# bkram/fmtuner-sdr

Measured on AMD Instinct MI355X. Metric: IQ MS/s demodulated per GPU (2.4 MS/s FM channels, stereo+RDS) at 1/2/4/8 MI355X, higher is better.
Workload: dtype f32 (FIR operands f16 hi+lo, f32 accumulate)

## Files before the change

fmtuner-sdr_amd/csrc/fmx_kernels.hip:

```cpp
#include <hip/hip_ext.h>
#include <hip/hip_fp16.h>
#include <hip/hip_runtime.h>

#include <cstddef>
#include <type_traits>

#include "fmx_internal.h"
#include "fmx_math.h"
#include "fmx_synth.h"


namespace fmx {

#define FE_T 768
#define FE_HALO_IQ 120
#define AU_T 768
#define AU_HALO 120
#define AU_RHALO 32
#define AU_MAXOUT 256

static constexpr float kPiF = 3.14159265358979323846f;

#define FMX_CONST __attribute__((address_space(4)))
template <typename T> __device__ __forceinline__ const FMX_CONST T *cptr(const T *p) {
// ... 743 lines not shown
      }
      keep[cntk++] = v;
    }
    __syncthreads();
    cntk = 0;
    uint8_t *dh = a.dec_hist + (size_t)c * 2 * FMX_MAX_DEC;
    for (int h = tid; h < L - 1; h += 256) {
      const uint16_t v = keep[cntk++];
      dh[2 * h] = (uint8_t)(v & 255);
      dh[2 * h + 1] = (uint8_t)(v >> 8);
    }
    if (tid == 0) {
      long nv = (long)dec_valid + total;
      a.dec_valid[c] = (int)(nv > (L - 1) ? (L - 1) : nv);
    }
  }
  if (demod) {
    for (int h = tid; h < FE_HALO_IQ; h += 256) {
      const float2 v = xin[h];
      a.iq_hist[(size_t)c * (FMX_IQ_MAXLEN - 1) + h] = float2_t{v.x, v.y};
    }
    if (tid == 0) {
      a.dc_v[2 * c] = sh->carry_i;
      a.dc_v[2 * c + 1] = sh->carry_q;
      a.fd_prev[2 * c] = sh->fd_re;
      a.fd_prev[2 * c + 1] = sh->fd_im;
      if (par.agc != 0) {
        a.agc[2 * c] = agc_g;
        a.agc[2 * c + 1] = agc_y2p;
      }
    }
  }
  if (hist_out) {
    float *hist = a.st_hist_wr + (size_t)c * FMX_HIST;
    for (int h = tid; h < FMX_HIST; h += 256) hist[h] = mx[h];
  }
  if (rds) {
    if (tid < 32) a.rds_hist[(size_t)c * 32 + tid] = rb[tid];
    if (tid == 0) a.rds_count[c] = sched_n;
  }
  FE_STAMP(6)
#ifdef FMX_STAMPS
  if (a.dbg && tid == 0)
    for (int k = 0; k < 8; ++k) atomicAdd(a.dbg + k, st_acc[k]);
#endif
#undef FE_STAMP
  if (tid == 0 && a.clip_out && a.in_mode != FE_IN_MPX)
    a.clip_out[c] = (n > 0) ? (float)sh->clip / (float)n : 0.0f;
  if (want_sig) fe_signal_sums(a, sig, sgp, c, lane, wave, tid);
}

__device__ __forceinline__ void dma_dword(const float *src, uint32_t lds) {
  unsigned keep;
  asm volatile("s_mov_b32 %0, m0\n\ts_mov_b32 m0, %2\n\ts_nop 0\n\tglobal_load_lds_dword %1, off\n\ts_mov_b32 m0, %0"
               : "=&s"(keep)
               : "v"(src), "s"(__builtin_amdgcn_readfirstlane(lds))
               : "memory");
}
__device__ __forceinline__ void dma_dword_s(const float *base, uint32_t voff, uint32_t lds) {
  __builtin_amdgcn_global_load_lds(reinterpret_cast<const char *>(base) + voff,
                                   (__attribute__((address_space(3))) void *)(uintptr_t)__builtin_amdgcn_readfirstlane(lds), 4, 0, 0);
}
__device__ __forceinline__ void dma_dwordx3(const float *src, uint32_t lds) {
  unsigned keep;
  asm volatile("s_mov_b32 %0, m0\n\ts_mov_b32 m0, %2\n\ts_nop 0\n\tglobal_load_lds_dwordx3 %1, off\n\ts_mov_b32 m0, %0"
               : "=&s"(keep)
               : "v"(src), "s"(__builtin_amdgcn_readfirstlane(lds))
               : "memory");
}
__device__ __forceinline__ uint32_t lds_addr(const void *p) {
  return __builtin_amdgcn_readfirstlane((uint32_t)(uintptr_t)(const __attribute__((address_space(3))) char *)p);
}
__device__ __forceinline__ void word_sincos(uint32_t theta, float *s, float *c) { fmx_word_sincos(theta, s, c); }

#include "fmx_pll.inc"

#define AU2_T 2048
#define AU2_PT 8
#define AU2_MAXOUT (AU2_T / 3 + 16)
#define AU_IMG (AU_HALO + AU2_T + 24)
#define AU_FN (AU_RHALO + AU2_T)
struct AuShared {
  float2 xf[AU_IMG > AU_FN ? AU_IMG : AU_FN] __attribute__((aligned(16)));
  float2 fh[AU_RHALO];
  float2 o[AU2_MAXOUT];
  float hT[FMX_AF_SUB][FMX_NPFB];
  float2 hf[AU_HALO];
  float ws[3][4][2];
  float iir[4];
  int eb, ee, count;
  uint32_t lrq[((2 * FMX_LR_QN + 63) / 64) * 64] __attribute__((aligned(16)));
};

template <int CTRL, int ROWS> __device__ __forceinline__ float dpp_or(float x, float id) {
  return __builtin_bit_cast(float, __builtin_amdgcn_update_dpp(__builtin_bit_cast(int, id), __builtin_bit_cast(int, x), CTRL,
                                                               ROWS, 0xF, false));
}
#define WAVE_AFF_STEP(CTRL, ROWS)                                                       \
  {                                                                                   \
    const float pA_ = dpp_or<CTRL, ROWS>(A, 1.0f), p1_ = dpp_or<CTRL, ROWS>(B1, 0.0f); \
    const float p2_ = dpp_or<CTRL, ROWS>(B2, 0.0f);                                     \
    B1 = A * p1_ + B1;                                                                \
    B2 = A * p2_ + B2;                                                                \
    A = A * pA_;                                                                      \
  }
__device__ __forceinline__ void wave_affine_scan(float &A, float &B1, float &B2) {
  WAVE_AFF_STEP(0x111, 0xF)
  WAVE_AFF_STEP(0x112, 0xF)
  WAVE_AFF_STEP(0x114, 0xF)
  WAVE_AFF_STEP(0x118, 0xF)
  WAVE_AFF_STEP(0x142, 0xA)
  WAVE_AFF_STEP(0x143, 0xC)
}
#undef WAVE_AFF_STEP
__device__ __forceinline__ void wave_affine_prev(float A, float B1, float B2, float &eA, float &e1, float &e2) {
  eA = dpp_or<0x138, 0xF>(A, 1.0f);
  e1 = dpp_or<0x138, 0xF>(B1, 0.0f);
  e2 = dpp_or<0x138, 0xF>(B2, 0.0f);
}

__device__ __forceinline__ void au_scan_prev(float A, float BL, float BR, float cl, float cr, float (*ws)[4][2],
                                             float &pl, float &pr) {
  const int tid = threadIdx.x, lane = tid & 63, wave = tid >> 6;
  wave_affine_scan(A, BL, BR);
  if (lane == 63) {
    ws[0][wave][0] = A;
    ws[1][wave][0] = BL;
    ws[2][wave][0] = BR;
  }
  float eA, eL, eR;
  wave_affine_prev(A, BL, BR, eA, eL, eR);
  __syncthreads();
  float vl = cl, vr = cr;
  for (int w = 0; w < wave; ++w) {
    vl = ws[0][w][0] * vl + ws[1][w][0];
    vr = ws[0][w][0] * vr + ws[2][w][0];
  }
  pl = eA * vl + eL;
  pr = eA * vr + eR;
  __syncthreads();
}

#ifndef FMX_AU_WPE
#define FMX_AU_WPE 1
#endif
__global__ __launch_bounds__(256) __attribute__((amdgpu_waves_per_eu(FMX_AU_WPE))) void k_audio(AudioArgs a) {
  extern __shared__ __align__(16) unsigned char au_smem[];
  AuShared &S = *reinterpret_cast<AuShared *>(au_smem);
  const int c = au_channel(blockIdx.x, a.C, a.in_tiled != 0);
  const int tid = threadIdx.x;
  const FmxDesign *__restrict__ D = a.des;
  const FmxChanParam par = a.par[c];
  const int n = a.n;
  const bool mono = (a.mode == 2 || a.mode == 3);
  const bool lrfir = (a.mode == 0 || a.mode == 4);
  const bool af = (a.mode != 4);
  const bool pipe_mono = (a.mode == 3);
  const int deemph = par.deemph;
  const float dalpha = (deemph == 0) ? D->deemph_alpha[0] : ((deemph == 1) ? D->deemph_alpha[1] : par.deemph_alpha);
  const bool de_on = deemph != 2;
  const float dc_alpha = mono ? 0.0008f : 0.005f;
  const float de_a1 = -(1.0f - dalpha);
  const float dc_a1 = -1.0f + dc_alpha;
  if (a.sig_out && blockIdx.x * 256 < (unsigned)a.C) {
    const int cs = blockIdx.x * 256 + tid;
    if (cs < a.C)
      signal_level_eval(a.sig_sums + 6 * (size_t)cs, a.sig_samples, a.sig_par + 4 * (size_t)cs,
                        a.sig_smooth + 2 * (size_t)cs, a.sig_out + cs);
  }
  float *lrh = a.lr_hist + (size_t)c * 2 * (FMX_LR_LEN - 1);
  float *win = mono ? a.mono_win + (size_t)c * 32 : a.af_win + (size_t)c * 2 * 32;
  float2 *const F = S.xf;
  float2 cx = make_float2(0.0f, 0.0f);
  if (lrfir && tid < AU_HALO) cx = make_float2(lrh[tid], lrh[(FMX_LR_LEN - 1) + tid]);
  if (af)
    for (int h = tid; h < AU_RHALO; h += 256) S.fh[h] = make_float2(win[h], mono ? 0.0f : win[32 + h]);
  float *iir = mono ? a.mono_iir + (size_t)c * 2 : a.af_iir + (size_t)c * 4;
  if (af && tid == 0) {
    if (mono) {
      S.iir[0] = iir[0];
      S.iir[1] = 0.0f;
      S.iir[2] = iir[1];
      S.iir[3] = 0.0f;
    } else {
      for (int k = 0; k < 4; ++k) S.iir[k] = iir[k];
    }
  }
  const FmxSched *sched = nullptr;
  int sched_n = 0;
  if (af) {
    const int g = a.group[c];
    sched = a.sched + (size_t)g * a.sched_stride;
    sched_n = a.sched_n[g];
    for (int k = tid; k < FMX_NPFB * FMX_AF_SUB; k += 256) {
      const int b = k / FMX_AF_SUB, nn = k % FMX_AF_SUB;
      S.hT[nn][b] = D->af_h[k];
    }
  }
  if (lrfir) {
    static_assert(FMX_LR_QN % 2 == 0, "dword window");
    const float *qs = reinterpret_cast<const float *>(&D->lr_q16[0][0][0]);
    for (int p = tid >> 6; p < (2 * FMX_LR_QN + 63) / 64; p += 4)
      dma_dword(qs + min(64 * p + (tid & 63), 2 * FMX_LR_QN - 1), lds_addr(&S.lrq[64 * p]));
  }
  if (tid == 0) {
    S.eb = 0;
    S.count = 0;
  }
  const bool tiled = a.in_tiled != 0;
  const float *inl = a.in_l + (tiled ? lr_tile_idx(c, 0, a.in_stride) : (size_t)c * a.in_stride);
  const float *inr = mono ? nullptr : a.in_r + (tiled ? lr_tile_idx(c, 0, a.in_stride) : (size_t)c * a.in_stride);
  auto ti = [&](int j) __attribute__((always_inline)) { return tiled ? (j >> 4) * 32 + (j & 15) : j; };
  const float sc = D->lr_scale;
  int mrem = 0, mtot = 0;
  if (a.mute) {
    mrem = a.mute[2 * c];
    mtot = a.mute[2 * c + 1];
  }
  const int mdone = (mtot > mrem) ? mtot - mrem : 0;
  const int mfade = max(1, min(a.mute_fade, mtot / 2));
  __syncthreads();
  for (int n0 = 0; n0 < n; n0 += AU2_T) {
    const int cnt = min(AU2_T, n - n0);
    FmxSched en3[3];
    if (af) {
      const int eb = S.eb;
#pragma unroll
      for (int k = 0; k < 3; ++k) {
        const int e = eb + tid + 256 * k;
        en3[k] = (e < sched_n) ? sched[e] : FmxSched{0xFFFF, 0.0f};
      }
    }
    {
      float vl[AU2_PT], vr[AU2_PT];
#pragma unroll
      for (int k = 0; k < AU2_PT; ++k) {
        const int j = tid + 256 * k;
        vl[k] = (j < cnt) ? inl[ti(n0 + j)] : 0.0f;
        vr[k] = (j < cnt && !mono) ? inr[ti(n0 + j)] : 0.0f;
      }
      if (lrfir) {
        _Float16 *im = reinterpret_cast<_Float16 *>(S.xf);
        auto put = [&](int i, float l, float r) __attribute__((always_inline)) {
          l *= 1024.0f;
          r *= 1024.0f;
          const _Float16 lh = (_Float16)l, rh = (_Float16)r;
          im[i] = lh;
          im[AU_IMG + i] = (_Float16)(l - (float)lh);
          im[2 * AU_IMG + i] = rh;
          im[3 * AU_IMG + i] = (_Float16)(r - (float)rh);
        };
        if (tid < AU_HALO) put(tid, cx.x, cx.y);
#pragma unroll
        for (int k = 0; k < AU2_PT; ++k) put(AU_HALO + tid + 256 * k, vl[k], vr[k]);
        if (tid < AU_IMG - AU_HALO - AU2_T) put(AU_HALO + AU2_T + tid, 0.0f, 0.0f);
#pragma unroll
        for (int k = 0; k < AU2_PT; ++k) {
          const int j = tid + 256 * k;
          if (j >= cnt - AU_HALO && j < cnt) S.hf[j - (cnt - AU_HALO)] = make_float2(vl[k], vr[k]);
        }
        if (tid < AU_HALO && tid >= cnt) S.hf[tid - cnt] = cx;
      } else {
#pragma unroll
        for (int k = 0; k < AU2_PT; ++k) {
          const int j = tid + 256 * k;
          if (j < cnt) F[AU_RHALO + j] = make_float2(vl[k], vr[k]);
        }
      }
      if (!lrfir && af && tid < AU_RHALO) F[tid] = S.fh[tid];
    }
    if (tid == 0) S.ee = S.eb;
    __syncthreads();
    if (lrfir) {
      typedef _Float16 f16x8_t __attribute__((ext_vector_type(8)));
      typedef float f32x4_t __attribute__((ext_vector_type(4)));
      typedef unsigned int u32x4 __attribute__((ext_vector_type(4)));
      const int lane = tid & 63, wave = tid >> 6, col = lane & 15, g = lane >> 4;
      const _Float16 *im = reinterpret_cast<const _Float16 *>(S.xf);
      const int xb = 16 * (32 * wave + col) + 8 * g;
      const f16x8_t *bLh = reinterpret_cast<const f16x8_t *>(im + xb);
      const f16x8_t *bLl = reinterpret_cast<const f16x8_t *>(im + AU_IMG + xb);
      const f16x8_t *bRh = reinterpret_cast<const f16x8_t *>(im + 2 * AU_IMG + xb);
      const f16x8_t *bRl = reinterpret_cast<const f16x8_t *>(im + 3 * AU_IMG + xb);
      const int qb = 8 * g + 15 - col, qc = qb & 1;
      const uint32_t *qh = &S.lrq[0] + qc * FMX_LR_QN + (qb - qc) / 2;
      const uint32_t *ql = qh + FMX_LR_QN / 2;
      auto frag = [&](int ks, const uint32_t *q) __attribute__((always_inline)) {
        return u32x4{q[16 * ks], q[16 * ks + 1], q[16 * ks + 2], q[16 * ks + 3]};
      };
      f32x4_t aL[2], aR[2];
      aL[0] = aL[1] = aR[0] = aR[1] = f32x4_t{0.0f, 0.0f, 0.0f, 0.0f};
      u32x4 ah = frag(0, qh), al = frag(0, ql);
#pragma unroll
      for (int ks = 0; ks < FMX_LR_KS; ++ks) {
        const f16x8_t ahi = __builtin_bit_cast(f16x8_t, ah), alo = __builtin_bit_cast(f16x8_t, al);
        if (ks + 1 < FMX_LR_KS) {
          ah = frag(ks + 1, qh);
          al = frag(ks + 1, ql);
        }
#pragma unroll
        for (int u = 0; u < 2; ++u) {
          const f16x8_t lh = bLh[32 * u + 4 * ks], ll = bLl[32 * u + 4 * ks];
          const f16x8_t rh = bRh[32 * u + 4 * ks], rl = bRl[32 * u + 4 * ks];
          aL[u] = __builtin_amdgcn_mfma_f32_16x16x32_f16(lh, ahi, aL[u], 0, 0, 0);
          aR[u] = __builtin_amdgcn_mfma_f32_16x16x32_f16(rh, ahi, aR[u], 0, 0, 0);
          aL[u] = __builtin_amdgcn_mfma_f32_16x16x32_f16(ll, ahi, aL[u], 0, 0, 0);
          aR[u] = __builtin_amdgcn_mfma_f32_16x16x32_f16(rl, ahi, aR[u], 0, 0, 0);
          aL[u] = __builtin_amdgcn_mfma_f32_16x16x32_f16(lh, alo, aL[u], 0, 0, 0);
          aR[u] = __builtin_amdgcn_mfma_f32_16x16x32_f16(rh, alo, aR[u], 0, 0, 0);
        }
      }
      if (tid < AU_HALO) cx = S.hf[tid];
      __syncthreads();
      if (af && tid < AU_RHALO) F[tid] = S.fh[tid];
      const float osc = sc * (1.0f / 4194304.0f);
#pragma unroll
      for (int u = 0; u < 2; ++u) {
#pragma unroll
        for (int i = 0; i < 4; ++i) {
          const int j = 256 * (2 * wave + u) + 16 * (4 * g + i) + col;
          const float2 y = make_float2(aL[u][i] * osc, aR[u][i] * osc);
          if (af) F[AU_RHALO + j] = y;
          if (a.lr_out_l && j < cnt) {
            a.lr_out_l[(size_t)c * a.lr_out_stride + n0 + j] = y.x;
            a.lr_out_r[(size_t)c * a.lr_out_stride + n0 + j] = y.y;
          }
        }
      }
    }
    __syncthreads();
    if (af) {
      const int eb = S.eb;
      int last = -1;
#pragma unroll
      for (int k = 0; k < 3; ++k) {
        const int e = eb + tid + 256 * k;
        if (e < sched_n && (en3[k].packed & 0xFFFF) < n0 + cnt) {
          const int i = (en3[k].packed & 0xFFFF) - n0;
          const int b = (en3[k].packed >> 16) & 0xFF;
          const bool boundary = (en3[k].packed >> 24) & 1;
          const int b0 = boundary ? FMX_NPFB - 1 : b, b1 = boundary ? 0 : b + 1;
          const int i0 = boundary ? i - 1 : i;
          float y0l = 0.0f, y0r = 0.0f, y1l = 0.0f, y1r = 0.0f;
          auto mac = [](float &y, float h, float x) __attribute__((always_inline)) {
            float t;
            asm("v_mul_f32 %0, %2, %3\n\tv_add_f32 %1, %1, %0" : "=&v"(t), "+v"(y) : "v"(h), "v"(x));
          };
#pragma unroll
          for (int m = 0; m < FMX_AF_SUB; ++m) {
            const float2 v0 = F[AU_RHALO + i0 - (FMX_AF_SUB - 1) + m];
            const float2 v1 = F[AU_RHALO + i - (FMX_AF_SUB - 1) + m];
            const float h0 = S.hT[FMX_AF_SUB - 1 - m][b0], h1 = S.hT[FMX_AF_SUB - 1 - m][b1];
            mac(y0l, h0, v0.x);
            mac(y0r, h0, v0.y);
            mac(y1l, h1, v1.x);
            mac(y1r, h1, v1.y);
          }
          const float mu = en3[k].mu, omu = 1.0f - mu;
          float yl, yr;
          asm("v_mul_f32 %0, %2, %3\n\tv_mul_f32 %1, %2, %4" : "=&v"(yl), "=&v"(yr) : "v"(omu), "v"(y0l), "v"(y0r));
          mac(yl, mu, y1l);
          mac(yr, mu, y1r);
          S.o[e - eb] = make_float2(yl, yr);
          last = e;
        }
      }
      if (last >= 0) atomicMax(&S.ee, last + 1);
      __syncthreads();
      const int m = S.ee - eb;
      float xl[3], xr[3];
      bool on[3];
#pragma unroll
      for (int k = 0; k < 3; ++k) {
        const int q = 3 * tid + k;
        on[k] = q < m;
        const float2 v = on[k] ? S.o[q] : make_float2(0.0f, 0.0f);
        xl[k] = v.x;
        xr[k] = v.y;
      }
      auto compose = [&](float a_, const float *bl, const float *br, float &A, float &BL, float &BR) {
        A = 1.0f;
        BL = 0.0f;
        BR = 0.0f;
#pragma unroll
        for (int k = 0; k < 3; ++k)
          if (on[k]) {
            BL = a_ * BL + bl[k];
            BR = a_ * BR + br[k];
            A = a_ * A;
          }
      };
      if (de_on) {
        float A, BL, BR, pl, pr;
        compose(-de_a1, xl, xr, A, BL, BR);
        au_scan_prev(A, BL, BR, S.iir[0], S.iir[1], S.ws, pl, pr);
#pragma unroll
        for (int k = 0; k < 3; ++k)
          if (on[k]) {
            const float vl = xl[k] - de_a1 * pl, vr = xr[k] - de_a1 * pr;
            if (3 * tid + k == m - 1) {
              S.iir[0] = vl;
              S.iir[1] = vr;
            }
            pl = vl;
            pr = vr;
            xl[k] = dalpha * vl;
            xr[k] = dalpha * vr;
          }
      }
      float A, BL, BR, ql, qr;
      compose(-dc_a1, xl, xr, A, BL, BR);
      au_scan_prev(A, BL, BR, S.iir[2], S.iir[3], S.ws, ql, qr);
      const int o0 = S.count;
#pragma unroll
      for (int k = 0; k < 3; ++k)
        if (on[k]) {
          const float vl = xl[k] - dc_a1 * ql, vr = xr[k] - dc_a1 * qr;
          float yl = vl - ql, yr = vr - qr;
          if (3 * tid + k == m - 1) {
            S.iir[2] = vl;
            S.iir[3] = vr;
          }
          ql = vl;
          qr = vr;
          if (pipe_mono) yl = yl * 0.5f;
          if (a.clamp) {
            yl = d_clamp(yl, -1.0f, 1.0f);
            yr = d_clamp(yr, -1.0f, 1.0f);
          }
          const int o = o0 + 3 * tid + k;
          if (o < mrem) {
            const int idx = mdone + o;
            float gain = 0.0f;
            if (idx < mfade) gain = 1.0f - ((float)idx / (float)mfade);
            else if (idx >= mtot - mfade) gain = (float)(mtot - idx) / (float)mfade;
            gain = d_clamp(gain, 0.0f, 1.0f);
            yl *= gain;
            yr *= gain;
          }
          if (o < a.cap) {
            a.out_l[(size_t)c * a.out_stride + o] = yl;
            if (pipe_mono) a.out_r[(size_t)c * a.out_stride + o] = yl;
            else if (!mono) a.out_r[(size_t)c * a.out_stride + o] = yr;
          }
        }
      __syncthreads();
      if (tid == 0) {
        S.count = o0 + m;
        S.eb = eb + m;
      }
    }
    {
      float2 cf = make_float2(0.0f, 0.0f);
      if (af && tid < AU_RHALO) cf = F[tid + cnt];
      __syncthreads();
      if (af && tid < AU_RHALO) S.fh[tid] = cf;
      __syncthreads();
    }
  }
  if (lrfir && tid < AU_HALO) {
    lrh[tid] = cx.x;
    lrh[(FMX_LR_LEN - 1) + tid] = cx.y;
  }
  if (af) {
    for (int h = tid; h < AU_RHALO; h += 256) {
      const float2 v = S.fh[h];
      win[h] = v.x;
      if (!mono) win[32 + h] = v.y;
    }
    if (tid == 0) {
      if (mono) {
        iir[0] = S.iir[0];
        iir[1] = S.iir[2];
      } else {
        for (int k = 0; k < 4; ++k) iir[k] = S.iir[k];
      }
    }
    const int nout = S.count < a.cap ? S.count : a.cap;
    if (tid == 0 && a.out_count) a.out_count[c] = nout;
    if (tid == 0 && a.mute && mrem > 0 && nout > 0) {
      const int mc = min(nout, mrem);
      a.mute[2 * c] = mrem - mc;
      if (mrem - mc == 0) a.mute[2 * c + 1] = 0;
    }
  }
}

enum { OA = 0, OB = 1, OC = 2, OCP = 3, OD = 4, OINV = 5 };
__device__ __forceinline__ int bs_block_number(int off) {
  return (off == OA) ? 0 : (off == OB) ? 1 : (off == OC || off == OCP) ? 2 : (off == OD) ? 3 : 0;
}
__device__ __forceinline__ int bs_next(int off) {
  return (off == OA) ? OB : (off == OB) ? OC : (off == OC || off == OCP) ? OD : OA;
}
__device__ __forceinline__ int bs_offset_for(uint32_t s) {
  switch (s) {
    case 0x3D8: return OA;
    case 0x3D4: return OB;
    case 0x25C: return OC;
    case 0x3CC: return OCP;
    case 0x258: return OD;
    default: return OINV;
  }
}
__constant__ uint32_t c_parity[26] = {0x200, 0x100, 0x080, 0x040, 0x020, 0x010, 0x008, 0x004, 0x002,
                                      0x001, 0x2DC, 0x16E, 0x0B7, 0x287, 0x39F, 0x313, 0x355, 0x376,
                                      0x1BB, 0x201, 0x3DC, 0x1EE, 0x0F7, 0x2A7, 0x38F, 0x31B};
__device__ __forceinline__ uint32_t bs_syndrome(uint32_t v) {
  uint32_t r = 0;
#pragma unroll
  for (int k = 0; k < 26; ++k) r ^= ((v >> k) & 1u) ? c_parity[25 - k] : 0u;
  return r;
}
__device__ __forceinline__ bool pulse_follows(uint32_t pos, int off, uint32_t opos, int ooff) {
  const uint32_t d = pos - opos;
  return d % 26 == 0 && d / 26 <= 6 && off != OINV && ooff != OINV &&
         ((uint32_t)bs_block_number(ooff) + d / 26) % 4 == (uint32_t)bs_block_number(off);
}

#define RDS_LPC 8
#define RDS_CPW (64 / RDS_LPC)
#define RDS_SYMQ 12
#ifndef RDS_PF
#define RDS_PF 3
#endif
#ifndef RDS_NR
#define RDS_NR 4
#endif
static_assert(RDS_PF < RDS_NR && (RDS_NR & (RDS_NR - 1)) == 0 && 3 * RDS_PF <= 63, "k_rds input ring");
static_assert(FMX_RDS_DECIM == 3 * RDS_LPC, "three samples per lane and decimation period");
struct RdsBits {
  float bi_prev_re, bi_prev_im, bi_even, bi_odd;
  uint32_t bi_clock, bi_polarity;
  int delta_prev;
  uint32_t bs_bitcount, bs_until_next, bs_reg, bs_err_mask_lo, bs_err_mask_hi;
  int bs_expected, bs_in_sync, bs_err_ptr;
  uint32_t bs_pulse_pos[4];
  int bs_pulse_off[4];
  uint32_t bs_blk_raw[4];
  uint16_t bs_blk_data[4];
  uint8_t bs_blk_flags[4];
  uint32_t bs_bits_since_lost;
};
struct RdsCold {
  RdsBits s;
  uint32_t pad_[(sizeof(RdsBits) / 4) % 2 == 0 ? 1 : 2];
};
static_assert((sizeof(RdsCold) / 4) % 2 == 1, "RdsCold must have an odd dword stride");
__device__ __forceinline__ void rds_bits_load(RdsBits &b, const FmxRdsState &g) {
  b.bi_prev_re = g.bi_prev_re;
  b.bi_prev_im = g.bi_prev_im;
  b.bi_even = g.bi_even;
  b.bi_odd = g.bi_odd;
  b.bi_clock = g.bi_clock;
  b.bi_polarity = g.bi_polarity;
  b.delta_prev = g.delta_prev;
  b.bs_bitcount = g.bs_bitcount;
  b.bs_until_next = g.bs_until_next;
  b.bs_reg = g.bs_reg;
  b.bs_err_mask_lo = g.bs_err_mask_lo;
  b.bs_err_mask_hi = g.bs_err_mask_hi;
// ... 1492 lines not shown
static thread_local hipEvent_t t_ev_start = nullptr, t_ev_stop = nullptr;
void set_launch_events(void *start, void *stop) {
  t_ev_start = static_cast<hipEvent_t>(start);
  t_ev_stop = static_cast<hipEvent_t>(stop);
}
template <typename K, typename... Args>
static int fmx_launch(K kernel, dim3 grid, dim3 block, size_t smem, hipStream_t st, Args... args) {
  hipEvent_t e0 = t_ev_start, e1 = t_ev_stop;
  t_ev_start = t_ev_stop = nullptr;
  if (e0 || e1) hipExtLaunchKernelGGL(kernel, grid, block, (uint32_t)smem, st, e0, e1, 0u, args...);
  else hipLaunchKernelGGL(kernel, grid, block, smem, st, args...);
  return hipGetLastError() == hipSuccess ? FMX_OK : FMX_E_HIP;
}

template <int M, int TPP, bool RS> static int fe8_launch_rs(const FeArgs &a, hipStream_t st) {
  static_assert(Fe8Layout<M, TPP, RS>::BYTES <= (160 * 1024 - 36864) / 2, "k_fe8: two workgroups per CU plus a k_pll / k_rds workgroup");
  static_assert(Fe8Layout<M, TPP, RS>::UOFF >= Fe8Layout<M, TPP, RS>::YB, "RDS copy above the IQ image");
  const size_t smem = (size_t)Fe8Layout<M, TPP, RS>::BYTES;
  static bool configured = false;
  if (!configured) {
    if (hipFuncSetAttribute(reinterpret_cast<const void *>(&k_fe8<M, TPP, RS>),
                            hipFuncAttributeMaxDynamicSharedMemorySize, (int)smem) != hipSuccess)
      return FMX_E_HIP;
    configured = true;
  }
  return fmx_launch(k_fe8<M, TPP, RS>, dim3(a.C), dim3(256), smem, st, a);
}
template <int M, int TPP> static int fe8_launch(const FeArgs &a, hipStream_t st) {
  if (a.pilot_out) return FMX_E_INVALID;
  if (a.rds_out && a.rds_win_out) return fe8_launch_rs<M, TPP, false>(a, st);
  return fe8_launch_rs<M, TPP, true>(a, st);
}

template <int M, int TPP, bool VEC> static int fe_launch(const FeArgs &a, hipStream_t st) {
  const size_t smem = (size_t)FeLayout<M, TPP, VEC>::BYTES;
  static bool configured = false;
  if (!configured) {
    if (hipFuncSetAttribute(reinterpret_cast<const void *>(&k_frontend<M, TPP, VEC>),
                            hipFuncAttributeMaxDynamicSharedMemorySize, (int)smem) != hipSuccess)
      return FMX_E_HIP;
    configured = true;
  }
  return fmx_launch(k_frontend<M, TPP, VEC>, dim3(a.C), dim3(256), smem, st, a);
}

}

namespace fmx {
static bool fe8_ok(const FeArgs &a, int M) {
  if (a.in_mode != FE_IN_U8_DECIM) return false;
  const bool aligned = ((((uintptr_t)a.iq) | (uintptr_t)a.iq_stride) & 15) == 0 && ((2L * a.n * M) & 15) == 0;
  return aligned && a.n >= FE8_MIN_N && (a.n & 3) == 0 && a.do_demod && !a.bb_out &&
         a.des_fs >= 190000;
}
bool frontend_is_fe8(const FeArgs &a, int M, int tpp) {
  return fe8_ok(a, M) && ((M == 10 && tpp == 28) || (M == 8 && tpp == 28) || (M == 4 && tpp == 20) ||
                               (M == 2 && tpp == 12));
}
int launch_frontend_m(const FeArgs &a, int M, int tpp, void *stream, bool vec) {
  hipStream_t st = static_cast<hipStream_t>(stream);
  if (a.in_mode != FE_IN_U8_DECIM) return fe_launch<1, 1, false>(a, st);
  const bool fe8 = fe8_ok(a, M);
  vec = vec && ((((uintptr_t)a.iq) | (uintptr_t)a.iq_stride) & 15) == 0 && ((2L * a.n * M) & 15) == 0;
  if (fe8) {
    if (M == 10 && tpp == 28) return fe8_launch<10, 28>(a, st);
    if (M == 8 && tpp == 28) return fe8_launch<8, 28>(a, st);
    if (M == 4 && tpp == 20) return fe8_launch<4, 20>(a, st);
    if (M == 2 && tpp == 12) return fe8_launch<2, 12>(a, st);
  }
  if (M == 10 && tpp == 28) return vec ? fe_launch<10, 28, true>(a, st) : fe_launch<10, 28, false>(a, st);
  if (M == 8 && tpp == 28) return vec ? fe_launch<8, 28, true>(a, st) : fe_launch<8, 28, false>(a, st);
  if (M == 4 && tpp == 20) return vec ? fe_launch<4, 20, true>(a, st) : fe_launch<4, 20, false>(a, st);
  if (M == 2 && tpp == 12) return vec ? fe_launch<2, 12, true>(a, st) : fe_launch<2, 12, false>(a, st);
  return FMX_E_INVALID;
}

int launch_pll(const PllArgs &a, void *stream) {
  const int n_cu = a.n_cu > 0 ? a.n_cu : 256;
  hipStream_t st = static_cast<hipStream_t>(stream);
  const int ch = 2 * ((a.C + 15) / 16) <= n_cu ? 16 : 24;
  if (ch == 16) return fmx_launch(k_pll<16>, dim3((a.C + 15) / 16), dim3(64 * PLL_WAVES(16)), 0, st, a);
  return fmx_launch(k_pll<24>, dim3((a.C + 23) / 24), dim3(64 * PLL_WAVES(24)), 0, st, a);
}
int launch_audio(const AudioArgs &a, void *stream) {
  return fmx_launch(k_audio, dim3(a.C), dim3(256), sizeof(AuShared), static_cast<hipStream_t>(stream), a);
}
#define PIL_TPW 4
#define PIL_SEG (4 * 256 * PIL_TPW)
#define PIL_QP ((2 * FMX_PILOT_QN + 63) / 64)
struct PilLds {
  _Float16 xh[FMX_HIST + PIL_SEG + 32] __attribute__((aligned(16)));
  _Float16 xl[FMX_HIST + PIL_SEG + 32] __attribute__((aligned(16)));
  uint32_t q[PIL_QP * 64] __attribute__((aligned(16)));
};
#ifndef FMX_PILOT_PRIO
#define FMX_PILOT_PRIO 0
#endif
__global__ __launch_bounds__(256) void k_pilot(PilotArgs a) {
  __shared__ PilLds L;
  if (FMX_PILOT_PRIO > 0) __builtin_amdgcn_s_setprio(FMX_PILOT_PRIO);
  typedef unsigned int u32x4 __attribute__((ext_vector_type(4)));
  typedef _Float16 f16x8_t __attribute__((ext_vector_type(8)));
  typedef _Float16 f16x4_t __attribute__((ext_vector_type(4)));
  typedef float f32x4_t __attribute__((ext_vector_type(4)));
  const FmxDesign *__restrict__ D = a.des;
  const int nseg = (a.n + PIL_SEG - 1) / PIL_SEG;
  const int units = a.C * nseg;
  const int per = (units + 7) / 8;
  const int u = (int)(blockIdx.x & 7) * per + (int)(blockIdx.x >> 3);
  if (u >= units) return;
  const int c = u / nseg, s0 = (u % nseg) * PIL_SEG;
  const int tid = threadIdx.x, lane = tid & 63, wave = tid >> 6;
  const int P8 = fir8_len(D->pilot_len);
  const int KSP = D->pilot_ks;
  const float *mrow = a.mpx + (size_t)c * a.mpx_stride;
  const float *hrow = a.st_hist_rd + (size_t)c * FMX_HIST + FMX_HIST;
  {
    static_assert(FMX_PILOT_QN % 2 == 0, "dword window");
    const float *qs = reinterpret_cast<const float *>(&D->pilot_q16[0][0][0]);
    for (int p = wave; p < PIL_QP; p += 4)
      dma_dword(qs + min(64 * p + lane, 2 * FMX_PILOT_QN - 1), lds_addr(&L.q[64 * p]));
  }
  const int i0 = FMX_HIST - (P8 - 1);
  constexpr int NPASS = (FMX_HIST + PIL_SEG + 32 + 1023) / 1024;
  float4 v[NPASS];
#pragma unroll
  for (int q = 0; q < NPASS; ++q) {
    const int i = i0 + 4 * tid + 1024 * q, s = s0 - FMX_HIST + i;
    if (i >= FMX_HIST + PIL_SEG + 32) continue;
    if (a.vec && s >= 0 && s + 4 <= a.n) {
      v[q] = *reinterpret_cast<const float4 *>(mrow + s);
    } else {
      float w[4];
#pragma unroll
      for (int k = 0; k < 4; ++k) w[k] = (s + k < 0) ? hrow[s + k] : (s + k < a.n ? mrow[s + k] : 0.0f);
      v[q] = make_float4(w[0], w[1], w[2], w[3]);
    }
  }
#pragma unroll
  for (int q = 0; q < NPASS; ++q) {
    const int i = i0 + 4 * tid + 1024 * q;
    if (i >= FMX_HIST + PIL_SEG + 32) continue;
    const float w[4] = {v[q].x, v[q].y, v[q].z, v[q].w};
    f16x4_t hv, lv;
#pragma unroll
    for (int k = 0; k < 4; ++k) {
      hv[k] = (_Float16)w[k];
      lv[k] = (_Float16)(w[k] - (float)hv[k]);
    }
    *reinterpret_cast<f16x4_t *>(&L.xh[i]) = hv;
    *reinterpret_cast<f16x4_t *>(&L.xl[i]) = lv;
  }
  asm volatile("s_waitcnt vmcnt(0)" ::: "memory");
  __syncthreads();
  const int col = lane & 15, g = lane >> 4;
  const int xb = FMX_HIST + 256 * PIL_TPW * wave + 16 * col - (P8 - 1) + 8 * g;
  const f16x8_t *bh = reinterpret_cast<const f16x8_t *>(&L.xh[xb]);
  const f16x8_t *bl = reinterpret_cast<const f16x8_t *>(&L.xl[xb]);
  const int qb = 8 * g + 15 - col, qc = qb & 1;
  const uint32_t *qh = &L.q[0] + qc * FMX_PILOT_QN + (qb - qc) / 2;
  const uint32_t *ql = qh + FMX_PILOT_QN / 2;
  auto frag = [&](int ks, int s) __attribute__((always_inline)) {
    const uint32_t *q = (s ? ql : qh) + 16 * ks;
    return u32x4{q[0], q[1], q[2], q[3]};
  };
  f32x4_t acc[PIL_TPW];
#pragma unroll
  for (int u = 0; u < PIL_TPW; ++u) acc[u] = f32x4_t{0.0f, 0.0f, 0.0f, 0.0f};
// ... 199 lines not shown
```

Baseline: 343,200.

## Template audio kernel on mode, vectorize tiled loads, prefetch chunks and drop barriers

```diff
diff --git a/fmtuner-sdr_amd/csrc/fmx_kernels.hip b/fmtuner-sdr_amd/csrc/fmx_kernels.hip
--- a/fmtuner-sdr_amd/csrc/fmx_kernels.hip
+++ b/fmtuner-sdr_amd/csrc/fmx_kernels.hip
@@ -849,13 +849,12 @@
 #define AU_FN (AU_RHALO + AU2_T)
 struct AuShared {
   float2 xf[AU_IMG > AU_FN ? AU_IMG : AU_FN] __attribute__((aligned(16)));
-  float2 fh[AU_RHALO];
   float2 o[AU2_MAXOUT];
   float hT[FMX_AF_SUB][FMX_NPFB];
   float2 hf[AU_HALO];
-  float ws[3][4][2];
+  float ws[2][3][4];
   float iir[4];
-  int eb, ee, count;
+  int ee;
   uint32_t lrq[((2 * FMX_LR_QN + 63) / 64) * 64] __attribute__((aligned(16)));
 };
 
@@ -886,125 +885,165 @@
   e2 = dpp_or<0x138, 0xF>(B2, 0.0f);
 }
 
-__device__ __forceinline__ void au_scan_prev(float A, float BL, float BR, float cl, float cr, float (*ws)[4][2],
+__device__ __forceinline__ void au_scan_prev(float A, float BL, float BR, float cl, float cr, float (*ws)[4],
                                              float &pl, float &pr) {
   const int tid = threadIdx.x, lane = tid & 63, wave = tid >> 6;
   wave_affine_scan(A, BL, BR);
   if (lane == 63) {
-    ws[0][wave][0] = A;
-    ws[1][wave][0] = BL;
-    ws[2][wave][0] = BR;
+    ws[0][wave] = A;
+    ws[1][wave] = BL;
+    ws[2][wave] = BR;
   }
   float eA, eL, eR;
   wave_affine_prev(A, BL, BR, eA, eL, eR);
   __syncthreads();
   float vl = cl, vr = cr;
   for (int w = 0; w < wave; ++w) {
-    vl = ws[0][w][0] * vl + ws[1][w][0];
-    vr = ws[0][w][0] * vr + ws[2][w][0];
+    vl = ws[0][w] * vl + ws[1][w];
+    vr = ws[0][w] * vr + ws[2][w];
   }
   pl = eA * vl + eL;
   pr = eA * vr + eR;
-  __syncthreads();
 }
 
 #ifndef FMX_AU_WPE
 #define FMX_AU_WPE 1
 #endif
+template <int MODE, bool VEC>
 __global__ __launch_bounds__(256) __attribute__((amdgpu_waves_per_eu(FMX_AU_WPE))) void k_audio(AudioArgs a) {
+  constexpr bool mono = (MODE == 2 || MODE == 3);
+  constexpr bool lrfir = (MODE == 0 || MODE == 4);
+  constexpr bool af = (MODE != 4);
+  constexpr bool pipe_mono = (MODE == 3);
+  static_assert(!VEC || lrfir, "pair tiles hold raw L/R");
+  static_assert(FMX_NPFB * FMX_AF_SUB == 3 * 256, "three resampler taps per thread");
+  typedef float f32x4_t __attribute__((ext_vector_type(4)));
   extern __shared__ __align__(16) unsigned char au_smem[];
   AuShared &S = *reinterpret_cast<AuShared *>(au_smem);
-  const int c = au_channel(blockIdx.x, a.C, a.in_tiled != 0);
+  const bool tiled = VEC || a.in_tiled != 0;
+  const int c = au_channel(blockIdx.x, a.C, tiled);
   const int tid = threadIdx.x;
   const FmxDesign *__restrict__ D = a.des;
-  const FmxChanParam par = a.par[c];
   const int n = a.n;
-  const bool mono = (a.mode == 2 || a.mode == 3);
-  const bool lrfir = (a.mode == 0 || a.mode == 4);
-  const bool af = (a.mode != 4);
-  const bool pipe_mono = (a.mode == 3);
-  const int deemph = par.deemph;
-  const float dalpha = (deemph == 0) ? D->deemph_alpha[0] : ((deemph == 1) ? D->deemph_alpha[1] : par.deemph_alpha);
-  const bool de_on = deemph != 2;
-  const float dc_alpha = mono ? 0.0008f : 0.005f;
-  const float de_a1 = -(1.0f - dalpha);
-  const float dc_a1 = -1.0f + dc_alpha;
   if (a.sig_out && blockIdx.x * 256 < (unsigned)a.C) {
     const int cs = blockIdx.x * 256 + tid;
     if (cs < a.C)
       signal_level_eval(a.sig_sums + 6 * (size_t)cs, a.sig_samples, a.sig_par + 4 * (size_t)cs,
                         a.sig_smooth + 2 * (size_t)cs, a.sig_out + cs);
   }
-  float *lrh = a.lr_hist + (size_t)c * 2 * (FMX_LR_LEN - 1);
-  float *win = mono ? a.mono_win + (size_t)c * 32 : a.af_win + (size_t)c * 2 * 32;
-  float2 *const F = S.xf;
-  float2 cx = make_float2(0.0f, 0.0f);
-  if (lrfir && tid < AU_HALO) cx = make_float2(lrh[tid], lrh[(FMX_LR_LEN - 1) + tid]);
-  if (af)
-    for (int h = tid; h < AU_RHALO; h += 256) S.fh[h] = make_float2(win[h], mono ? 0.0f : win[32 + h]);
-  float *iir = mono ? a.mono_iir + (size_t)c * 2 : a.af_iir + (size_t)c * 4;
-  if (af && tid == 0) {
-    if (mono) {
-      S.iir[0] = iir[0];
-      S.iir[1] = 0.0f;
-      S.iir[2] = iir[1];
-      S.iir[3] = 0.0f;
-    } else {
-      for (int k = 0; k < 4; ++k) S.iir[k] = iir[k];
-    }
-  }
-  const FmxSched *sched = nullptr;
-  int sched_n = 0;
-  if (af) {
-    const int g = a.group[c];
-    sched = a.sched + (size_t)g * a.sched_stride;
-    sched_n = a.sched_n[g];
-    for (int k = tid; k < FMX_NPFB * FMX_AF_SUB; k += 256) {
-      const int b = k / FMX_AF_SUB, nn = k % FMX_AF_SUB;
-      S.hT[nn][b] = D->af_h[k];
-    }
-  }
   if (lrfir) {
     static_assert(FMX_LR_QN % 2 == 0, "dword window");
     const float *qs = reinterpret_cast<const float *>(&D->lr_q16[0][0][0]);
     for (int p = tid >> 6; p < (2 * FMX_LR_QN + 63) / 64; p += 4)
       dma_dword(qs + min(64 * p + (tid & 63), 2 * FMX_LR_QN - 1), lds_addr(&S.lrq[64 * p]));
   }
-  if (tid == 0) {
-    S.eb = 0;
-    S.count = 0;
-  }
-  const bool tiled = a.in_tiled != 0;
+  int grp = 0;
+  if (af) grp = a.group[c];
+  const FmxChanParam par = a.par[c];
+  const float dalpha50 = D->deemph_alpha[0], dalpha75 = D->deemph_alpha[1];
+  const float sc = D->lr_scale;
+  float *lrh = a.lr_hist + (size_t)c * 2 * (FMX_LR_LEN - 1);
+  float *win = mono ? a.mono_win + (size_t)c * 32 : a.af_win + (size_t)c * 2 * 32;
+  float *iir = mono ? a.mono_iir + (size_t)c * 2 : a.af_iir + (size_t)c * 4;
+  float2 *const F = S.xf;
+  float2 cx = make_float2(0.0f, 0.0f);
+  if (lrfir) {
+    const int h = min(tid, AU_HALO - 1);
+    cx = make_float2(lrh[h], lrh[(FMX_LR_LEN - 1) + h]);
+  }
+  float2 cf = make_float2(0.0f, 0.0f);
+  float iv[4] = {0.0f, 0.0f, 0.0f, 0.0f}, hq[3] = {0.0f, 0.0f, 0.0f};
+  if (af) {
+    const int h = tid & (AU_RHALO - 1);
+    cf.x = win[h];
+    if (!mono) cf.y = win[32 + h];
+    iv[0] = iir[0];
+    if (mono) {
+      iv[2] = iir[1];
+    } else {
+      iv[1] = iir[1];
+      iv[2] = iir[2];
+      iv[3] = iir[3];
+    }
+#pragma unroll
+    for (int k = 0; k < 3; ++k) hq[k] = D->af_h[tid + 256 * k];
+  }
+  const int *mp = a.mute ? a.mute + 2 * c : reinterpret_cast<const int *>(a.par + c);
+  const int mw0 = mp[0], mw1 = mp[1];
+  const int mrem = a.mute ? mw0 : 0, mtot = a.mute ? mw1 : 0;
   const float *inl = a.in_l + (tiled ? lr_tile_idx(c, 0, a.in_stride) : (size_t)c * a.in_stride);
   const float *inr = mono ? nullptr : a.in_r + (tiled ? lr_tile_idx(c, 0, a.in_stride) : (size_t)c * a.in_stride);
   auto ti = [&](int j) __attribute__((always_inline)) { return tiled ? (j >> 4) * 32 + (j & 15) : j; };
-  const float sc = D->lr_scale;
-  int mrem = 0, mtot = 0;
-  if (a.mute) {
-    mrem = a.mute[2 * c];
-    mtot = a.mute[2 * c + 1];
-  }
+  auto own = [&](int q) __attribute__((always_inline)) {
+    return VEC ? 4 * tid + 1024 * (q >> 2) + (q & 3) : tid + 256 * q;
+  };
+  float nxl[AU2_PT], nxr[AU2_PT];
+  auto load_chunk = [&](int n0) __attribute__((always_inline)) {
+    const int cnt = min(AU2_T, n - n0);
+    if constexpr (VEC) {
+#pragma unroll
+      for (int k = 0; k < AU2_PT / 4; ++k) {
+        const int j = own(4 * k), t = (j < cnt) ? n0 + j : 0;
+        const f32x4_t l = *reinterpret_cast<const f32x4_t *>(inl + ti(t));
+        const f32x4_t r = *reinterpret_cast<const f32x4_t *>(inr + ti(t));
+#pragma unroll
+        for (int e = 0; e < 4; ++e) {
+          nxl[4 * k + e] = l[e];
+          nxr[4 * k + e] = r[e];
+        }
+      }
+    } else {
+#pragma unroll
+      for (int q = 0; q < AU2_PT; ++q) {
+        const int j = own(q), t = (j < cnt) ? n0 + j : 0;
+        nxl[q] = inl[ti(t)];
+        nxr[q] = mono ? 0.0f : inr[ti(t)];
+      }
+    }
+  };
+  load_chunk(0);
+  __builtin_amdgcn_sched_barrier(0);
+  const FmxSched *sched = nullptr;
+  int sched_n = 0;
+  FmxSched en3[3] = {};
+  auto load_sched = [&](int eb) __attribute__((always_inline)) {
+#pragma unroll
+    for (int k = 0; k < 3; ++k) en3[k] = sched[max(min(eb + tid + 256 * k, a.sched_stride - 1), 0)];
+  };
+  if (af) {
+    sched = a.sched + (size_t)grp * a.sched_stride;
+    sched_n = a.sched_n[grp];
+    load_sched(0);
+  }
+  const int deemph = par.deemph;
+  const float dalpha = (deemph == 0) ? dalpha50 : ((deemph == 1) ? dalpha75 : par.deemph_alpha);
+  const bool de_on = deemph != 2;
+  const float dc_alpha = mono ? 0.0008f : 0.005f;
+  const float de_a1 = -(1.0f - dalpha);
+  const float dc_a1 = -1.0f + dc_alpha;
   const int mdone = (mtot > mrem) ? mtot - mrem : 0;
   const int mfade = max(1, min(a.mute_fade, mtot / 2));
+  if (af) {
+#pragma unroll
+    for (int k = 0; k < 3; ++k) {
+      const int q = tid + 256 * k;
+      S.hT[q % FMX_AF_SUB][q / FMX_AF_SUB] = hq[k];
+    }
+    if (tid == 0)
+      for (int k = 0; k < 4; ++k) S.iir[k] = iv[k];
+  }
+  int eb = 0, count = 0;
   __syncthreads();
   for (int n0 = 0; n0 < n; n0 += AU2_T) {
     const int cnt = min(AU2_T, n - n0);
-    FmxSched en3[3];
-    if (af) {
-      const int eb = S.eb;
-#pragma unroll
-      for (int k = 0; k < 3; ++k) {
-        const int e = eb + tid + 256 * k;
-        en3[k] = (e < sched_n) ? sched[e] : FmxSched{0xFFFF, 0.0f};
-      }
-    }
     {
+      if (n0 > 0) load_chunk(n0);
       float vl[AU2_PT], vr[AU2_PT];
 #pragma unroll
-      for (int k = 0; k < AU2_PT; ++k) {
-        const int j = tid + 256 * k;
-        vl[k] = (j < cnt) ? inl[ti(n0 + j)] : 0.0f;
-        vr[k] = (j < cnt && !mono) ? inr[ti(n0 + j)] : 0.0f;
+      for (int q = 0; q < AU2_PT; ++q) {
+        const bool in = own(q) < cnt;
+        vl[q] = in ? nxl[q] : 0.0f;
+        vr[q] = (in && !mono) ? nxr[q] : 0.0f;
       }
       if (lrfir) {
         _Float16 *im = reinterpret_cast<_Float16 *>(S.xf);
@@ -1018,25 +1057,47 @@
           im[3 * AU_IMG + i] = (_Float16)(r - (float)rh);
         };
         if (tid < AU_HALO) put(tid, cx.x, cx.y);
-#pragma unroll
-        for (int k = 0; k < AU2_PT; ++k) put(AU_HALO + tid + 256 * k, vl[k], vr[k]);
+        if constexpr (VEC) {
+          typedef _Float16 f16x4_t __attribute__((ext_vector_type(4)));
+          static_assert((2 * AU_HALO) % 8 == 0 && (2 * AU_IMG) % 8 == 0, "8-B image writes");
+#pragma unroll
+          for (int k = 0; k < AU2_PT / 4; ++k) {
+            f16x4_t lh, ll, rh, rl;
+#pragma unroll
+            for (int e = 0; e < 4; ++e) {
+              const float l = vl[4 * k + e] * 1024.0f, r = vr[4 * k + e] * 1024.0f;
+              lh[e] = (_Float16)l;
+              rh[e] = (_Float16)r;
+              ll[e] = (_Float16)(l - (float)lh[e]);
+              rl[e] = (_Float16)(r - (float)rh[e]);
+            }
+            const int i = AU_HALO + own(4 * k);
+            *reinterpret_cast<f16x4_t *>(im + i) = lh;
+            *reinterpret_cast<f16x4_t *>(im + AU_IMG + i) = ll;
+            *reinterpret_cast<f16x4_t *>(im + 2 * AU_IMG + i) = rh;
+            *reinterpret_cast<f16x4_t *>(im + 3 * AU_IMG + i) = rl;
+          }
+        } else {
+#pragma unroll
+          for (int q = 0; q < AU2_PT; ++q) put(AU_HALO + own(q), vl[q], vr[q]);
+        }
         if (tid < AU_IMG - AU_HALO - AU2_T) put(AU_HALO + AU2_T + tid, 0.0f, 0.0f);
 #pragma unroll
-        for (int k = 0; k < AU2_PT; ++k) {
-          const int j = tid + 256 * k;
-          if (j >= cnt - AU_HALO && j < cnt) S.hf[j - (cnt - AU_HALO)] = make_float2(vl[k], vr[k]);
+        for (int q = 0; q < AU2_PT; ++q) {
+          const int j = own(q);
+          if (j >= cnt - AU_HALO && j < cnt) S.hf[j - (cnt - AU_HALO)] = make_float2(vl[q], vr[q]);
         }
         if (tid < AU_HALO && tid >= cnt) S.hf[tid - cnt] = cx;
       } else {
 #pragma unroll
-        for (int k = 0; k < AU2_PT; ++k) {
-          const int j = tid + 256 * k;
-          if (j < cnt) F[AU_RHALO + j] = make_float2(vl[k], vr[k]);
-        }
-      }
-      if (!lrfir && af && tid < AU_RHALO) F[tid] = S.fh[tid];
-    }
-    if (tid == 0) S.ee = S.eb;
+        for (int q = 0; q < AU2_PT; ++q) {
+          const int j = own(q);
+          if (j < cnt) F[AU_RHALO + j] = make_float2(vl[q], vr[q]);
+        }
+        if (tid < AU_RHALO) F[tid] = cf;
+      }
+    }
+    if (tid == 0) S.ee = eb;
     __syncthreads();
     if (lrfir) {
       typedef _Float16 f16x8_t __attribute__((ext_vector_type(8)));
@@ -1079,7 +1140,7 @@
       }
       if (tid < AU_HALO) cx = S.hf[tid];
       __syncthreads();
-      if (af && tid < AU_RHALO) F[tid] = S.fh[tid];
+      if (af && tid < AU_RHALO) F[tid] = cf;
       const float osc = sc * (1.0f / 4194304.0f);
 #pragma unroll
       for (int u = 0; u < 2; ++u) {
@@ -1088,7 +1149,7 @@
           const int j = 256 * (2 * wave + u) + 16 * (4 * g + i) + col;
           const float2 y = make_float2(aL[u][i] * osc, aR[u][i] * osc);
           if (af) F[AU_RHALO + j] = y;
-          if (a.lr_out_l && j < cnt) {
+          if (MODE == 4 && a.lr_out_l && j < cnt) {
             a.lr_out_l[(size_t)c * a.lr_out_stride + n0 + j] = y.x;
             a.lr_out_r[(size_t)c * a.lr_out_stride + n0 + j] = y.y;
           }
@@ -1097,7 +1158,6 @@
     }
     __syncthreads();
     if (af) {
-      const int eb = S.eb;
       int last = -1;
 #pragma unroll
       for (int k = 0; k < 3; ++k) {
@@ -1135,6 +1195,8 @@
       if (last >= 0) atomicMax(&S.ee, last + 1);
       __syncthreads();
       const int m = S.ee - eb;
+      if (tid < AU_RHALO) cf = F[tid + cnt];
+      load_sched(eb + m);
       float xl[3], xr[3];
       bool on[3];
 #pragma unroll
@@ -1160,7 +1222,7 @@
       if (de_on) {
         float A, BL, BR, pl, pr;
         compose(-de_a1, xl, xr, A, BL, BR);
-        au_scan_prev(A, BL, BR, S.iir[0], S.iir[1], S.ws, pl, pr);
+        au_scan_prev(A, BL, BR, S.iir[0], S.iir[1], S.ws[0], pl, pr);
 #pragma unroll
         for (int k = 0; k < 3; ++k)
           if (on[k]) {
@@ -1177,8 +1239,8 @@
       }
       float A, BL, BR, ql, qr;
       compose(-dc_a1, xl, xr, A, BL, BR);
-      au_scan_prev(A, BL, BR, S.iir[2], S.iir[3], S.ws, ql, qr);
-      const int o0 = S.count;
+      au_scan_prev(A, BL, BR, S.iir[2], S.iir[3], S.ws[1], ql, qr);
+      const int o0 = count;
 #pragma unroll
       for (int k = 0; k < 3; ++k)
         if (on[k]) {
@@ -1211,18 +1273,8 @@
             else if (!mono) a.out_r[(size_t)c * a.out_stride + o] = yr;
           }
         }
-      __syncthreads();
-      if (tid == 0) {
-        S.count = o0 + m;
-        S.eb = eb + m;
-      }
-    }
-    {
-      float2 cf = make_float2(0.0f, 0.0f);
-      if (af && tid < AU_RHALO) cf = F[tid + cnt];
-      __syncthreads();
-      if (af && tid < AU_RHALO) S.fh[tid] = cf;
-      __syncthreads();
+      count += m;
+      eb += m;
     }
   }
   if (lrfir && tid < AU_HALO) {
@@ -1230,11 +1282,11 @@
     lrh[(FMX_LR_LEN - 1) + tid] = cx.y;
   }
   if (af) {
-    for (int h = tid; h < AU_RHALO; h += 256) {
-      const float2 v = S.fh[h];
-      win[h] = v.x;
-      if (!mono) win[32 + h] = v.y;
-    }
+    if (tid < AU_RHALO) {
+      win[tid] = cf.x;
+      if (!mono) win[32 + tid] = cf.y;
+    }
+    __syncthreads();
     if (tid == 0) {
       if (mono) {
         iir[0] = S.iir[0];
@@ -1243,7 +1295,7 @@
         for (int k = 0; k < 4; ++k) iir[k] = S.iir[k];
       }
     }
-    const int nout = S.count < a.cap ? S.count : a.cap;
+    const int nout = count < a.cap ? count : a.cap;
     if (tid == 0 && a.out_count) a.out_count[c] = nout;
     if (tid == 0 && a.mute && mrem > 0 && nout > 0) {
       const int mc = min(nout, mrem);
@@ -2902,8 +2954,24 @@
   if (ch == 16) return fmx_launch(k_pll<16>, dim3((a.C + 15) / 16), dim3(64 * PLL_WAVES(16)), 0, st, a);
   return fmx_launch(k_pll<24>, dim3((a.C + 23) / 24), dim3(64 * PLL_WAVES(24)), 0, st, a);
 }
+template <int MODE> static int launch_audio_mode(const AudioArgs &a, hipStream_t st) {
+  if constexpr (MODE == 0 || MODE == 4) {
+    const bool vec = a.in_tiled && a.in_stride % 16 == 0 &&
+                     ((reinterpret_cast<uintptr_t>(a.in_l) | reinterpret_cast<uintptr_t>(a.in_r)) & 15) == 0;
+    if (vec) return fmx_launch(k_audio<MODE, true>, dim3(a.C), dim3(256), sizeof(AuShared), st, a);
+  }
+  return fmx_launch(k_audio<MODE, false>, dim3(a.C), dim3(256), sizeof(AuShared), st, a);
+}
 int launch_audio(const AudioArgs &a, void *stream) {
-  return fmx_launch(k_audio, dim3(a.C), dim3(256), sizeof(AuShared), static_cast<hipStream_t>(stream), a);
+  hipStream_t st = static_cast<hipStream_t>(stream);
+  switch (a.mode) {
+    case 0: return launch_audio_mode<0>(a, st);
+    case 1: return launch_audio_mode<1>(a, st);
+    case 2: return launch_audio_mode<2>(a, st);
+    case 3: return launch_audio_mode<3>(a, st);
+    case 4: return launch_audio_mode<4>(a, st);
+  }
+  return FMX_E_INVALID;
 }
 #define PIL_TPW 4
 #define PIL_SEG (4 * 256 * PIL_TPW)
```

Measured after the change: 346,600 (median of 6 runs). Within noise of the previous version (+1.0%).
